# marianaGarcez/SpatialFlink

Measured on AMD Instinct MI355X. Metric: points/sec per window (kNN k=50, range r) at 1/2/4/8 MI355X; % HBM roofline, higher is better.
Workload: dtype f64

## Files before the change

### spatialflink_amd/csrc/gf_internal.hpp

```cpp
#pragma once

#include <hip/hip_runtime.h>

#include <cstdint>
#include <string>
#include <vector>

#include "../../include/geoflink_hip.h"
#include "gf_text.hpp"
#include "gf_numerics.hpp"

struct gf_ctx {
  int device = 0;
  hipStream_t stream = nullptr;
  hipStream_t own_stream = nullptr;
  std::string last_error;
  int timing = 0;
  int timing_period = 1;
  int64_t timing_seq[GF_K_COUNT] = {};
  struct Ev { hipEvent_t a, b; int kid; };
  std::vector<Ev> pending;
  std::vector<hipEvent_t> pool;
  double acc_ms[GF_K_COUNT] = {};
  int64_t acc_n[GF_K_COUNT] = {};
// ... 131 lines not shown
};

struct KnnSampleArgs {
  const double* x;
  const double* y;
  int64_t n;
  double qx, qy;
  QueryRect qr;
  double r, s_r;
  int32_t k;
  int metric;
  int use_hint;
  KnnState* st;
};

struct PolyView {
  const int32_t* ring_off;
  const int32_t* vert_off;
  const double* vx;
  const double* vy;
  const double* ring_env;
  int metric;
  const uint8_t* rect;
};

struct KnnPolyArgs {
  const double* x;
  const double* y;
  const int64_t* objID;
  int64_t begin, end;
  QueryRect qr;
  PolyView poly;
  double bbox[4];
  int approx;
  double r;
  int32_t k;
  int use_state;
  int use_hint;
  KnnState* st;
  double* cand_d;
  uint32_t* cand_i;
  int64_t* cand_o;
  unsigned long long cap;
  uint32_t* maybe_i;
};

struct KnnSelectArgs {
  KnnState* st;
  const double* cand_d;
  const uint32_t* cand_i;
  const int64_t* cand_o;
  unsigned long long cap;
  int use_state;
  double T;
  double r;
  int32_t k;
  int write_hint;
  int64_t idx_base;
  void* result;
};

constexpr int kRangeMaxParts = 4096;
constexpr int kRangeTicketSlot = 2 * kRangeMaxParts;

struct RangeArgs {
  const double* x;
// ... 335 lines not shown
  int64_t* c_maxLen;
  int64_t* c_maxKey;
  int64_t* all_key;
  int64_t* all_len;
};
hipError_t launch_tagg(gf_ctx* ctx, int stage, const TaggArgs& a);

hipError_t launch_knn_sample(gf_ctx* ctx, const KnnSampleArgs& a);
hipError_t launch_knn_scan(gf_ctx* ctx, const KnnScanArgs& a, int blocks, int unroll, int nt);
hipError_t launch_knn_select(gf_ctx* ctx, const KnnSelectArgs& a);
struct KnnLargeArgs {
  const double* cd;
  const int64_t* co;
  const uint32_t* ci;
  uint32_t* perm;
  int64_t m;
  int field;
  uint32_t* keys;
  uint32_t* out;
  uint32_t* cnt;
  int pass;
  unsigned long long* lane_count;
  unsigned long long* lane_maybe;
  int32_t k;
  double T;
  int64_t idx_base;
  void* result;
};
hipError_t launch_knn_large(gf_ctx* ctx, int op, const KnnLargeArgs& a);
constexpr int32_t kMaxKLarge = 1 << 24;
int knn_exact_record(gf_knn_plan* P, const gf_points* pts, void* result);

hipError_t launch_knn_poly_sample(gf_ctx* ctx, const KnnPolyArgs& a);
hipError_t launch_knn_poly_scan(gf_ctx* ctx, const KnnPolyArgs& a, int blocks);
struct KnnSelectArgs;
struct KnnMergeArgs;
hipError_t launch_knn_poly_fused(gf_ctx* ctx, const KnnPolyArgs& a, const KnnSelectArgs& prev, int has_prev,
                                 int blocks, const KnnMergeArgs* merge);
__host__ __device__ inline size_t merge_any_hash(int64_t e) {
  size_t h = 1024;
  while (h < 2 * (size_t)e) h <<= 1;
  return h;
}
__host__ __device__ inline size_t merge_any_bytes(int32_t nrec, int32_t k) {
  const int64_t e = (int64_t)nrec * k;
  return ((size_t)e * 24 + merge_any_hash(e) * 12 + 255) & ~(size_t)255;
}
hipError_t launch_knn_merge(gf_ctx* ctx, int32_t k, const void* records, int32_t nrec, size_t rec_stride,
                            int32_t nwin, size_t win_stride, void* result, size_t res_stride, int foreign,
                            void* scratch);
__host__ __device__ inline size_t str_side_off(int32_t k) { return ((size_t)4 * (k + 1) + 7) & ~(size_t)7; }
__host__ __device__ inline size_t str_record_bytes(int32_t k, int64_t cap) {
  return 32 + (size_t)24 * k + 16 + str_side_off(k) + (((size_t)cap + 7) & ~(size_t)7);
}
__host__ __device__ inline size_t strmerge_pow2(int64_t e) {
  size_t p = 2;
  while (p < (size_t)e) p <<= 1;
  return p;
}
__host__ __device__ inline size_t strmerge_bytes(int32_t nrec, int32_t k) {
  const int64_t e = (int64_t)nrec * k;
  return ((size_t)e * 40 + strmerge_pow2(e) * 4 + strmerge_pow2(2 * e) * 8 + (size_t)k * 16 + 1024) & ~(size_t)255;
}
hipError_t launch_knn_attach_strings(gf_ctx* ctx, int32_t k, const unsigned long long* idmap, const char* arena,
                                     int64_t dict_size, const void* records, int32_t nrec, int64_t cap, void* out);
hipError_t launch_knn_merge_strings(gf_ctx* ctx, int32_t k, int64_t cap, const void* records, int32_t nrec,
                                    size_t rec_stride, int32_t nwin, size_t win_stride, void* results, void* scratch);
constexpr int kMaxMergeRecs = 64;
struct KnnRecList {
  const char* rec[kMaxMergeRecs];
};
// ... 233 lines not shown
  gf_grid grid{};
  double qx = 0, qy = 0, r = 0;
  int32_t k = 0;
  int metric = 0;
  gf::QueryRect qr{};
  struct Lane {
    gf::KnnState* st = nullptr;
    double* cand_d = nullptr;
    uint32_t* cand_i = nullptr;
    int64_t* cand_o = nullptr;
  } lane[6];
  int64_t cap = 0;
  int pipeline = 1;
  uint64_t seq = 0;
  int pend_lane = -1;
  int lane_warm[6] = {0, 0, 0, 0, 0, 0};
  void* pend_result = nullptr;
  int64_t pend_idx_base = 0;
  struct Pend {
    int lane;
    void* result;
    int64_t idx_base;
    uint64_t seq;
  };
  Pend pq[3];
  int npq = 0;
  int use_hint = 1;
  int64_t idx_base = 0;
  void* tmp_result = nullptr;
  void* host_result = nullptr;
  int scan_blocks = 0;
  int scan_unroll = 2;
  int scan_nt = 1;
  int large = 0;
  int poly = 0, approx = 0;
  int32_t* ring_off = nullptr;
  int32_t* vert_off = nullptr;
  double* vx = nullptr;
  double* vy = nullptr;
  double* ring_env = nullptr;
  double bbox[4] = {0, 0, 0, 0};
  uint32_t* maybe_i[3] = {nullptr, nullptr, nullptr};
  int64_t maybe_cap = 0;
};

struct gf_window {
  gf_ctx* ctx = nullptr;
  int64_t capacity = 0, n = 0;
  double* x = nullptr;
  double* y = nullptr;
  int64_t* objID = nullptr;
  int64_t* ts = nullptr;
  bool has_objid = false, has_ts = false;
  const int64_t* objid_mapped = nullptr;
  hipStream_t copy = nullptr;
  hipEvent_t ready = nullptr, fence_main = nullptr, fence_aux = nullptr, fence_aux2 = nullptr;
  bool pending = false;
};
```

### spatialflink_amd/csrc/k_knn.hip

```cpp
#define GF_TU_NAME k_knn_hip
#include "gf_buildtag.hpp"

#include <type_traits>

#include "gf_geom.hpp"
#include "gf_internal.hpp"

namespace gf {

__device__ __forceinline__ bool classify_cg(const QueryRect& q, double px, double py) {
  const double xs = (px == px) ? px : q.minX;
  const double ys = (py == py) ? py : q.minY;
  const bool inG = q.g_any && in_iv(q.gx, xs) && in_iv(q.gy, ys);
  return inG || (in_iv(q.cgx, xs) && in_iv(q.cgy, ys));
}

template <int METRIC>
__device__ __forceinline__ bool knn_pass(double qx, double qy, const QueryRect& qr, double px, double py,
                                         double sp, double T) {
  const double dx = qx - px, dy = qy - py;
  const double s = dx * dx + dy * dy;
  if (!(s <= sp)) return false;
  if (!classify_cg(qr, px, py)) return false;
  return METRIC == 0 ? true : fdlibm_hypot(dx, dy) <= T;
// ... 1126 lines not shown
  for (int j = threadIdx.x; j < kDistBins; j += kBlock) lh[j] = 0u;
  __syncthreads();
  const int64_t n = a.end - a.begin;
  const int64_t stride = n / gridDim.x;
  const int64_t p0 = a.begin + (int64_t)blockIdx.x * stride;
  const int64_t bbase = dist_bin_base(a.r);
  for (int u = threadIdx.x; u < kSamplePerBlock; u += kBlock) {
    const double px = a.x[p0 + u], py = a.y[p0 + u];
    double d;
    if (poly_pass(a, px, py, a.r, d)) atomicAdd(&lh[dist_bin(d, bbase)], 1u);
  }
  sample_finish(a.st, lh, a.k, a.r, a.poly.metric, bbase);
}

__device__ __forceinline__ bool poly_maybe(const KnnPolyArgs& a, double px, double py, double T) {
  if (!classify_cg(a.qr, px, py)) return false;
  return !(px == px && py == py && env_far(a.bbox, px, py, T));
}

__device__ __forceinline__ void maybe_append(const KnnPolyArgs& a, bool c, int64_t i) {
  const uint64_t m = __ballot(c);
  if (m == 0) return;
  const int lane = threadIdx.x & 63;
  const int leader = __ffsll((unsigned long long)m) - 1;
  unsigned long long base = 0;
  if (lane == leader) base = atomicAdd(&a.st->maybe, (unsigned long long)__popcll(m));
  base = __shfl(base, leader, 64);
  if (c) {
    const unsigned long long pos = base + (unsigned long long)__popcll(m & ((1ull << lane) - 1ull));
    if (pos < a.cap) a.maybe_i[pos] = (uint32_t)i;
  }
}

__device__ __forceinline__ void knn_poly_scan_body(const KnnPolyArgs& a, double T, int64_t bid, int64_t nblk) {
  const int lane = threadIdx.x & 63;
  const int64_t stride = nblk * kBlock;
  const int64_t pb = a.begin >> 1, pe = a.end >> 1;
  for (int64_t p = pb + bid * kBlock + threadIdx.x; p - lane < pe; p += stride) {
    const bool in = p < pe;
    dbl2 xv = {0.0, 0.0}, yv = {0.0, 0.0};
    if (in) {
      xv = __builtin_nontemporal_load(reinterpret_cast<const dbl2*>(a.x) + p);
      yv = __builtin_nontemporal_load(reinterpret_cast<const dbl2*>(a.y) + p);
    }
    const bool c0 = in && poly_maybe(a, xv.x, yv.x, T);
    const bool c1 = in && poly_maybe(a, xv.y, yv.y, T);
    if (__ballot(c0 || c1) == 0) continue;
    maybe_append(a, c0, 2 * p);
    maybe_append(a, c1, 2 * p + 1);
  }
  if ((a.end & 1) && bid == 0 && threadIdx.x < 64) {
    const int64_t i = a.end - 1;
    maybe_append(a, lane == 0 && poly_maybe(a, a.x[i], a.y[i], T), i);
  }
}

__global__ __launch_bounds__(kBlock) void knn_poly_scan_kernel(KnnPolyArgs a) {
  knn_poly_scan_body(a, a.use_state ? a.st->T : a.r, blockIdx.x, gridDim.x);
}

__global__ __launch_bounds__(kBlock) void knn_poly_fused_kernel(KnnPolyArgs a, KnnSelectArgs prev, int has_prev,
                                                                KnnMergeArgs m) {
  __shared__ SelLite L;
  if (blockIdx.x == 0) {
    if (has_prev) knn_select_body<SelLite, false>(prev, L);
    if (m.nrec > 0) {
      __threadfence();
      __syncthreads();
      const ListRecs src{&m.list};
      knn_merge_body(prev.k, src, m.nrec, m.result, L);
    }
    return;
  }
  double T;
  if (a.use_state == 2) {
    T = a.st->T;
  } else {
    const double h = a.st->hint_T;
    T = (h > 0.0 && h < a.r) ? h : a.r;
    if (blockIdx.x == 1 && threadIdx.x == 0) a.st->T = T;
  }
  knn_poly_scan_body(a, T, blockIdx.x - 1, gridDim.x - 1);
}

__global__ __launch_bounds__(kBlock) void knn_poly_refine_kernel(KnnPolyArgs a) {
  const double T = a.use_state ? a.st->T : a.r;
  const unsigned long long nm = a.st->maybe;
  if (nm > a.cap) {
    if (blockIdx.x == 0 && threadIdx.x == 0) atomicAdd(&a.st->count, nm);
    return;
  }
  const int lane = threadIdx.x & 63;
  const int64_t stride = (int64_t)gridDim.x * kBlock;
  for (int64_t j = (int64_t)blockIdx.x * kBlock + threadIdx.x; j - lane < (int64_t)nm; j += stride) {
    const bool in = j < (int64_t)nm;
    const int64_t i = in ? (int64_t)a.maybe_i[j] : 0;
    double d = 0.0;
    bool c = false;
    if (in) {
      const double px = a.x[i], py = a.y[i];
      d = a.approx ? point_bbox_distance(px, py, a.bbox) : polygon_distance(px, py, a.poly, 0);
      c = d <= T;
    }
    const uint64_t m = __ballot(c);
    if (m == 0) continue;
    const int leader = __ffsll((unsigned long long)m) - 1;
    unsigned long long base = 0;
    if (lane == leader) base = atomicAdd(&a.st->count, (unsigned long long)__popcll(m));
    base = __shfl(base, leader, 64);
    if (c) {
      const unsigned long long pos = base + (unsigned long long)__popcll(m & ((1ull << lane) - 1ull));
      if (pos < a.cap) {
        a.cand_d[pos] = d;
        a.cand_i[pos] = (uint32_t)i;
        a.cand_o[pos] = a.objID[i];
      }
    }
  }
}

hipError_t launch_knn_poly_sample(gf_ctx* ctx, const KnnPolyArgs& a) {
  KTimer t(ctx, GF_K_KNN_SAMPLE);
  hipLaunchKernelGGL(knn_poly_sample_kernel, dim3(kSampleBlocks), dim3(kBlock), 0, ctx->stream, a);
  return hipGetLastError();
}

hipError_t launch_knn_poly_fused(gf_ctx* ctx, const KnnPolyArgs& a, const KnnSelectArgs& prev, int has_prev,
                                 int blocks, const KnnMergeArgs* merge) {
  KnnMergeArgs m{};
  if (merge && has_prev) m = *merge;
  {
    KTimer t(ctx, GF_K_KNN_SCAN);
    hipLaunchKernelGGL(knn_poly_fused_kernel, dim3(blocks + 1), dim3(kBlock), 0, ctx->stream, a, prev, has_prev, m);
  }
  KnnPolyArgs r = a;
  r.use_state = 1;
  hipLaunchKernelGGL(knn_poly_refine_kernel, dim3(256), dim3(kBlock), 0, ctx->stream, r);
  return hipGetLastError();
}

hipError_t launch_knn_poly_scan(gf_ctx* ctx, const KnnPolyArgs& a, int blocks) {
  {
    KTimer t(ctx, GF_K_KNN_SCAN);
    hipLaunchKernelGGL(knn_poly_scan_kernel, dim3(blocks), dim3(kBlock), 0, ctx->stream, a);
  }
  hipLaunchKernelGGL(knn_poly_refine_kernel, dim3(256), dim3(kBlock), 0, ctx->stream, a);
  return hipGetLastError();
}

struct StrSide {
  int32_t status;
  int32_t n;
  int64_t nbytes;
};
__device__ __forceinline__ StrSide* side_of(void* rec, int32_t k) {
  return reinterpret_cast<StrSide*>((char*)rec + 32 + (size_t)24 * k);
}
__device__ __forceinline__ uint32_t* side_off(void* rec, int32_t k) { return reinterpret_cast<uint32_t*>(side_of(rec, k) + 1); }
__device__ __forceinline__ char* side_bytes(void* rec, int32_t k) { return (char*)side_off(rec, k) + str_side_off(k); }
__device__ __forceinline__ bool dict_key(int64_t o) { return o < GF_OBJID_NUMERIC_MIN; }

template <int NT>
__device__ __forceinline__ uint32_t block_excl(uint32_t v, uint32_t* excl, uint32_t* ws) {
  const int lane = threadIdx.x & 63, w = threadIdx.x >> 6;
  uint32_t inc = v;
#pragma unroll
  for (int o = 1; o < 64; o <<= 1) {
    const uint32_t t = __shfl_up(inc, o, 64);
    if (lane >= o) inc += t;
  }
  if (lane == 63) ws[w] = inc;
  __syncthreads();
  uint32_t before = 0, tot = 0;
#pragma unroll
  for (int i = 0; i < NT / 64; ++i) {
    before += i < w ? ws[i] : 0u;
    tot += ws[i];
  }
  *excl = before + inc - v;
  __syncthreads();
  return tot;
// ... 228 lines not shown
```

### spatialflink_amd/csrc/knn.cpp

```cpp
#define GF_TU_NAME knn_cpp
#include "gf_buildtag.hpp"

#include <hip/hip_runtime.h>

#include <initializer_list>
#include <iterator>
#include <limits>
#include <unordered_set>

#include "gf_host.hpp"

using namespace gf;

extern "C" size_t gf_knn_result_bytes(int32_t k) {
  return sizeof(gf_knn_header) + (size_t)(k > 0 ? k : 0) * (sizeof(double) + 2 * sizeof(int64_t));
}

extern "C" void gf_knn_plan_destroy(gf_knn_plan* P) {
  if (!P) return;
  hipSetDevice(P->ctx->device);
  hipStreamSynchronize(P->ctx->stream);
  for (auto& L : P->lane) {
    if (L.st) hipFree(L.st);
    if (L.cand_d) hipFree(L.cand_d);
// ... 88 lines not shown
    double mnx = poly->vx[v0], mxx = mnx, mny = poly->vy[v0], mxy = mny;
    for (int32_t v = v0 + 1; v < v1; ++v) {
      mnx = std::min(mnx, poly->vx[v]); mxx = std::max(mxx, poly->vx[v]);
      mny = std::min(mny, poly->vy[v]); mxy = std::max(mxy, poly->vy[v]);
    }
    renv[4 * j] = mnx; renv[4 * j + 1] = mxx; renv[4 * j + 2] = mny; renv[4 * j + 3] = mxy;
  }
  P->bbox[0] = renv[0]; P->bbox[1] = renv[2]; P->bbox[2] = renv[1]; P->bbox[3] = renv[3];
  const int32_t gl = guaranteed_layers(g->cellLength, r), cl = candidate_layers(g->cellLength, r);
  const int64_t bx0 = cell_index(P->bbox[0], g->minX, g->cellLength), bx1 = cell_index(P->bbox[2], g->minX, g->cellLength);
  const int64_t by0 = cell_index(P->bbox[1], g->minY, g->cellLength), by1 = cell_index(P->bbox[3], g->minY, g->cellLength);
  const double nan = std::numeric_limits<double>::quiet_NaN();
  const int64_t n1 = g->n - 1;
  QueryRect q;
  q.minX = g->minX;
  q.minY = g->minY;
  if (cl > 0) {
    q.cgx = axis_iv(std::max<int64_t>(bx0 - cl, 0), std::min<int64_t>(bx1 + cl, n1), g->minX, g->cellLength);
    q.cgy = axis_iv(std::max<int64_t>(by0 - cl, 0), std::min<int64_t>(by1 + cl, n1), g->minY, g->cellLength);
  } else {
    q.cgx = q.cgy = {nan, nan};
  }
  if (gl > 0) {
    q.gx = axis_iv(std::max<int64_t>(bx0 - gl, 0), std::min<int64_t>(bx1 + gl, n1), g->minX, g->cellLength);
    q.gy = axis_iv(std::max<int64_t>(by0 - gl, 0), std::min<int64_t>(by1 + gl, n1), g->minY, g->cellLength);
  } else if (gl == 0) {
    q.gx = axis_iv(bx0, bx1, g->minX, g->cellLength);
    q.gy = axis_iv(by0, by1, g->minY, g->cellLength);
  } else {
    q.gx = q.gy = {nan, nan};
  }
  q.g_any = (gl >= 0) && !std::isnan(q.gx.lo) && !std::isnan(q.gy.lo);
  P->qr = q;
  const int32_t nverts = poly->vert_off[nrings];
  std::vector<int32_t> ro = {0, nrings}, vo(poly->vert_off, poly->vert_off + nrings + 1);
  std::vector<double> vx(poly->vx, poly->vx + nverts), vy(poly->vy, poly->vy + nverts);
  if ((st = upload(ctx, &P->ring_off, ro)) || (st = upload(ctx, &P->vert_off, vo)) || (st = upload(ctx, &P->vx, vx)) ||
      (st = upload(ctx, &P->vy, vy)) || (st = upload(ctx, &P->ring_env, renv))) {
    gf_knn_plan_destroy(P);
    return st;
  }
  *out = P;
  return GF_OK;
}

extern "C" int gf_knn_plan_set_capacity(gf_knn_plan* P, int64_t cap) {
  if (!P || cap < 2 || cap > (int64_t)1 << 31) return GF_ERR_ARG;
  int st = bind(P->ctx);
  if (st) return st;
  int fs = gf_knn_plan_flush(P);
  if (fs) return fs;
  hipStreamSynchronize(P->ctx->stream);
  return knn_alloc_candidates(P, cap & ~(int64_t)1);
}

extern "C" int gf_knn_plan_set_tuning(gf_knn_plan* P, int32_t scan_blocks, int32_t unroll, int32_t nontemporal) {
  if (!P || scan_blocks < 0 || unroll < 1 || unroll > 8) return GF_ERR_ARG;
  P->scan_blocks = scan_blocks;
  P->scan_unroll = unroll;
  P->scan_nt = nontemporal != 0;
  return GF_OK;
}

extern "C" int gf_knn_plan_set_index_base(gf_knn_plan* P, int64_t base) {
  if (!P || base < 0) return GF_ERR_ARG;
  P->idx_base = base;
  return GF_OK;
}

static int scan_blocks_for(gf_knn_plan* P, int64_t n) {
  int blocks = P->scan_blocks;
  if (blocks <= 0) {
    blocks = stream_blocks(P->ctx, (n + 1) / 2);
    blocks = std::min(blocks, P->ctx->num_cus * 4);
  }
  return blocks;
}

static KnnScanArgs scan_args(gf_knn_plan* P, int j, const gf_points* pts, int64_t begin, int64_t end, int use_state) {
  const gf_knn_plan::Lane& L = P->lane[j];
  KnnScanArgs s{};
  s.x = pts->x; s.y = pts->y; s.objID = pts->objID; s.begin = begin; s.end = end;
  s.qx = P->qx; s.qy = P->qy; s.qr = P->qr;
  s.T = P->r; s.s_pre = s_prefilter(P->r, P->metric);
  s.use_state = use_state; s.metric = P->metric; s.st = L.st;
  s.cand_d = L.cand_d; s.cand_i = L.cand_i; s.cand_o = L.cand_o; s.cap = (unsigned long long)P->cap;
  return s;
}

static KnnSelectArgs select_args(gf_knn_plan* P, int j, int use_state, int write_hint, void* result,
                                 int64_t idx_base) {
  const gf_knn_plan::Lane& L = P->lane[j];
  KnnSelectArgs q{};
  q.st = L.st; q.cand_d = L.cand_d; q.cand_i = L.cand_i; q.cand_o = L.cand_o;
  q.cap = (unsigned long long)P->cap;
  q.use_state = use_state; q.T = P->r; q.r = P->r; q.k = P->k; q.result = result;
  q.write_hint = write_hint; q.idx_base = idx_base;
  return q;
}

static KnnPolyArgs poly_args(gf_knn_plan* P, int j, const gf_points* pts, int64_t begin, int64_t end, int use_state,
                             int use_hint) {
  const gf_knn_plan::Lane& L = P->lane[j];
  KnnPolyArgs a{};
  a.x = pts->x; a.y = pts->y; a.objID = pts->objID; a.begin = begin; a.end = end;
  a.qr = P->qr;
  a.poly = PolyView{P->ring_off, P->vert_off, P->vx, P->vy, P->ring_env, P->metric};
  for (int i = 0; i < 4; ++i) a.bbox[i] = P->bbox[i];
  a.approx = P->approx; a.r = P->r; a.k = P->k; a.use_state = use_state; a.use_hint = use_hint;
  a.st = L.st; a.cand_d = L.cand_d; a.cand_i = L.cand_i; a.cand_o = L.cand_o; a.cap = (unsigned long long)P->cap;
  a.maybe_i = P->maybe_i[P->pipeline >= 3 ? j % (P->pipeline - 1) : j];
  return a;
}

static int poly_buffers(gf_knn_plan* P) {
  if (P->maybe_cap >= P->cap) return GF_OK;
  GF_HIP_CHECK(P->ctx, hipStreamSynchronize(P->ctx->stream));
  if (int e = sync_aux(P->ctx)) return e;
  for (auto& m : P->maybe_i) {
    if (m) hipFree(m);
    m = nullptr;
    GF_HIP_CHECK(P->ctx, hipMalloc(&m, sizeof(uint32_t) * (size_t)P->cap));
  }
  P->maybe_cap = P->cap;
  return GF_OK;
}

static int knn_scan_select(gf_knn_plan* P, int j, const gf_points* pts, int64_t begin, int64_t end, int use_state,
                           int write_hint, void* result) {
  gf_ctx* ctx = P->ctx;
  if (P->poly) {
    int st = poly_buffers(P);
    if (st) return st;
    const KnnPolyArgs a = poly_args(P, j, pts, begin, end, use_state, 0);
    GF_HIP_CHECK(ctx, launch_knn_poly_scan(ctx, a, scan_blocks_for(P, (end - begin + 1) / 2)));
    GF_HIP_CHECK(ctx, launch_knn_select(ctx, select_args(P, j, use_state, write_hint, result, P->idx_base)));
    return GF_OK;
  }
  const KnnScanArgs s = scan_args(P, j, pts, begin, end, use_state);
  GF_HIP_CHECK(ctx, launch_knn_scan(ctx, s, scan_blocks_for(P, end - begin), P->scan_unroll, P->scan_nt));
  GF_HIP_CHECK(ctx, launch_knn_select(ctx, select_args(P, j, use_state, write_hint, result, P->idx_base)));
  return GF_OK;
}

static int knn_large(gf_knn_plan* P, const gf_points* pts, void* result) {
  gf_ctx* ctx = P->ctx;
  int st;
  const int64_t n = pts->n;
  if (P->cap < n && (st = knn_alloc_candidates(P, n))) return st;
  if (P->poly) {
    if ((st = poly_buffers(P))) return st;
    GF_HIP_CHECK(ctx, launch_knn_poly_scan(ctx, poly_args(P, 0, pts, 0, n, 0, 0), scan_blocks_for(P, (n + 1) / 2)));
  } else {
    const KnnScanArgs s = scan_args(P, 0, pts, 0, n, 0);
    GF_HIP_CHECK(ctx, launch_knn_scan(ctx, s, scan_blocks_for(P, n), P->scan_unroll, P->scan_nt));
  }
  const gf_knn_plan::Lane& L = P->lane[0];
  const int64_t mm = std::max<int64_t>(n, 1);
  const int nb = radix_blocks(ctx, mm);
  const int64_t mat = (int64_t)256 * nb;
  Arena ar;
  uint32_t *keys[2], *perm[2], *cnt, *m, *ms;
  ar.take(keys[0], mm); ar.take(keys[1], mm);
  ar.take(perm[0], mm); ar.take(perm[1], mm);
  ar.take(cnt, 2); ar.take(m, mat); ar.take(ms, mat + 1);
  if ((st = ar.alloc(ctx))) return st;
  KnnLargeArgs a{};
  a.cd = L.cand_d; a.co = L.cand_o; a.ci = L.cand_i; a.k = P->k; a.T = P->r; a.idx_base = P->idx_base;
  a.result = result; a.m = mm; a.cnt = cnt;
  a.lane_count = &L.st->count; a.lane_maybe = &L.st->maybe;
  GF_HIP_CHECK(ctx, launch_knn_large(ctx, 5, a));
  int cur = 0;
  auto sort_by = [&](int pass, std::initializer_list<int> fields) -> int {
    for (int f : fields) {
      a.perm = perm[cur]; a.field = f; a.keys = keys[0]; a.pass = pass;
      GF_HIP_CHECK(ctx, launch_knn_large(ctx, 1, a));
      for (int p = 0; p < 4; ++p) {
        RadixArgs r{};
        r.tile = radix_tile();
        r.n = mm; r.n_dev = a.cnt + pass;
        r.kin = keys[p & 1]; r.vin = perm[cur];
        r.kout = keys[(p + 1) & 1]; r.vout = perm[cur ^ 1];
        r.shift = p * 8; r.bits = 8; r.nblk = nb; r.M = m; r.Ms = ms;
        GF_HIP_CHECK(ctx, launch_radix(ctx, 0, r, nb));
        if (int e = scan1(ctx, m, mat, ms)) return e;
// ... 51 lines not shown
    const uint64_t kseq = P->seq++;
    const int S = P->pipeline >= 3 ? P->pipeline - 1 : 1, j = (int)(kseq % (uint64_t)S);
    hipStream_t main = ctx->stream;
    ctx->stream = knn_stream(ctx, main, j);
    const bool staged = pts->n >= kSampleMinN;
    int rc = staged ? knn_launch_sample(P, j, pts, P->use_hint) : GF_OK;
    if (rc == GF_OK) rc = knn_scan_select(P, j, pts, 0, pts->n, staged ? 1 : 0, staged && P->use_hint, result);
    ctx->stream = main;
    return rc;
  }
  if (P->pipeline >= 3) {
    if (P->poly && (st = poly_buffers(P))) return st;
    const uint64_t S = (uint64_t)(P->pipeline - 1), kseq = P->seq++;
    const int j = (int)(kseq % (2 * S));
    hipStream_t main = ctx->stream;
    ctx->stream = knn_stream(ctx, main, (int)(kseq % S));
    int rc = GF_OK;
    do {
      const bool sample = pts->n >= kSampleMinN && (!P->use_hint || !P->lane_warm[j]);
      if (sample && (rc = knn_launch_sample(P, j, pts, 0))) break;
      P->lane_warm[j] = 1;
      KnnSelectArgs q{};
      int has_prev = 0;
      if (P->npq > 0 && P->pq[0].seq + S == kseq) {
        const gf_knn_plan::Pend e = P->pq[0];
        q = select_args(P, e.lane, 1, P->use_hint, e.result, e.idx_base);
        has_prev = 1;
        for (int t = 1; t < P->npq; ++t) P->pq[t - 1] = P->pq[t];
        --P->npq;
      }
      hipError_t he;
      if (P->poly)
        he = launch_knn_poly_fused(ctx, poly_args(P, j, pts, 0, pts->n, sample ? 2 : 1, 0), q, has_prev,
                                   scan_blocks_for(P, (pts->n + 1) / 2), nullptr);
      else
        he = launch_knn_fused(ctx, scan_args(P, j, pts, 0, pts->n, sample ? 2 : 1), q, has_prev,
                              scan_blocks_for(P, pts->n), P->scan_unroll, P->scan_nt, merge);
      if (he != hipSuccess) { rc = hip_err(ctx, he, "launch_knn_fused"); break; }
      P->pq[P->npq++] = gf_knn_plan::Pend{j, result, P->idx_base, kseq};
    } while (0);
    ctx->stream = main;
    return rc;
  }
  if (P->pipeline == 2) {
    const int j = (int)(P->seq++ & 1);
    if (P->poly && (st = poly_buffers(P))) return st;
    const bool sample = pts->n >= kSampleMinN && (!P->use_hint || !P->lane_warm[j]);
    if (sample && (st = knn_launch_sample(P, j, pts, 0))) return st;
    P->lane_warm[j] = 1;
    const int use_state = sample ? 2 : 1;
    KnnSelectArgs q{};
    const int has_prev = P->pend_lane >= 0;
    if (has_prev) q = select_args(P, P->pend_lane, 1, P->use_hint, P->pend_result, P->pend_idx_base);
    const bool fold = merge && merge->nrec > 0 && has_prev && P->k <= kFusedMergeMaxK;
    if (P->poly)
      GF_HIP_CHECK(ctx, launch_knn_poly_fused(ctx, poly_args(P, j, pts, 0, pts->n, use_state, 0), q, has_prev,
                                             scan_blocks_for(P, (pts->n + 1) / 2), fold ? merge : nullptr));
    else
      GF_HIP_CHECK(ctx, launch_knn_fused(ctx, scan_args(P, j, pts, 0, pts->n, use_state), q, has_prev,
                                         scan_blocks_for(P, pts->n), P->scan_unroll, P->scan_nt,
                                         fold ? merge : nullptr));
    *merged = fold ? 1 : 0;
    P->pend_lane = j;
    P->pend_result = result;
    P->pend_idx_base = P->idx_base;
    return GF_OK;
  }
  const bool staged = pts->n >= kSampleMinN;
  if (staged && (st = knn_launch_sample(P, 0, pts, P->use_hint))) return st;
  return knn_scan_select(P, 0, pts, 0, pts->n, staged ? 1 : 0, staged && P->use_hint, result);
}

extern "C" int gf_knn_plan_flush(gf_knn_plan* P) {
  if (!P) return GF_ERR_ARG;
  if (P->pipeline >= 3) {
    if (P->npq == 0) return P->k > kFusedSelectMaxK ? gf_ctx_join(P->ctx) : GF_OK;
    gf_ctx* ctx = P->ctx;
    int st = bind(ctx);
    if (st) return st;
    hipStream_t main = ctx->stream;
    for (int e = 0; e < P->npq; ++e) {
      const gf_knn_plan::Pend& w = P->pq[e];
      ctx->stream = knn_stream(ctx, main, (int)(w.seq % (uint64_t)(P->pipeline - 1)));
      hipError_t he = launch_knn_select(ctx, select_args(P, w.lane, 1, P->use_hint, w.result, w.idx_base));
      ctx->stream = main;
      if (he != hipSuccess) return hip_err(ctx, he, "launch_knn_select");
    }
    P->npq = 0;
    return gf_ctx_join(ctx);
  }
// ... 182 lines not shown
```

Before: 768.7 billion.

## Filter polygon kNN scan on x first, loading y only for surviving lanes

The polygon kNN scan now checks each point's x coordinate against the query grid intervals and the polygon bbox band before loading y. It only issues y loads for tiles where some lane survives, which cuts HBM reads when x alone rejects most points. The scan body is also templated on an unroll factor and a nontemporal flag, with software prefetch of the next x tile. When T equals the full radius r, it falls back to the old path that loads both coordinates. The x-band test uses a small relative slack, so correctness depends on that tolerance staying conservative.

```diff
diff --git a/spatialflink_amd/csrc/gf_internal.hpp b/spatialflink_amd/csrc/gf_internal.hpp
--- a/spatialflink_amd/csrc/gf_internal.hpp
+++ b/spatialflink_amd/csrc/gf_internal.hpp
@@ -588,11 +588,11 @@
 int knn_exact_record(gf_knn_plan* P, const gf_points* pts, void* result);
 
 hipError_t launch_knn_poly_sample(gf_ctx* ctx, const KnnPolyArgs& a);
-hipError_t launch_knn_poly_scan(gf_ctx* ctx, const KnnPolyArgs& a, int blocks);
+hipError_t launch_knn_poly_scan(gf_ctx* ctx, const KnnPolyArgs& a, int blocks, int unroll, int nt);
 struct KnnSelectArgs;
 struct KnnMergeArgs;
 hipError_t launch_knn_poly_fused(gf_ctx* ctx, const KnnPolyArgs& a, const KnnSelectArgs& prev, int has_prev,
-                                 int blocks, const KnnMergeArgs* merge);
+                                 int blocks, int unroll, int nt, const KnnMergeArgs* merge);
 __host__ __device__ inline size_t merge_any_hash(int64_t e) {
   size_t h = 1024;
   while (h < 2 * (size_t)e) h <<= 1;
@@ -892,6 +892,8 @@
   int scan_blocks = 0;
   int scan_unroll = 2;
   int scan_nt = 1;
+  int poly_unroll = 1;
+  int poly_nt = 0;
   int large = 0;
   int poly = 0, approx = 0;
   int32_t* ring_off = nullptr;
diff --git a/spatialflink_amd/csrc/k_knn.hip b/spatialflink_amd/csrc/k_knn.hip
--- a/spatialflink_amd/csrc/k_knn.hip
+++ b/spatialflink_amd/csrc/k_knn.hip
@@ -1182,7 +1182,56 @@
   }
 }
 
-__device__ __forceinline__ void knn_poly_scan_body(const KnnPolyArgs& a, double T, int64_t bid, int64_t nblk) {
+struct PolyBand {
+  double T1;
+  double S;
+};
+__device__ __forceinline__ PolyBand poly_band(const KnnPolyArgs& a, double T) {
+  PolyBand b;
+  b.T1 = T * (1.0 + 1e-8);
+  b.S = fabs(a.bbox[0]) + fabs(a.bbox[1]) + fabs(a.bbox[2]) + fabs(a.bbox[3]);
+  return b;
+}
+__device__ __forceinline__ bool poly_x_maybe(const KnnPolyArgs& a, const PolyBand& b, double px) {
+  const bool num = px == px;
+  const double xs = num ? px : a.qr.minX;
+  if (!in_iv(a.qr.cgx, xs) && !(a.qr.g_any && in_iv(a.qr.gx, xs))) return false;
+  const double dx = px < a.bbox[0] ? a.bbox[0] - px : (px > a.bbox[2] ? px - a.bbox[2] : 0.0);
+  return !(num && dx > b.T1 + (fabs(px) + b.S) * 1e-11);
+}
+__device__ __forceinline__ uint32_t poly_x_mask(const KnnPolyArgs& a, const PolyBand& b, const dbl2& xv) {
+  return (uint32_t)poly_x_maybe(a, b, xv.x) | ((uint32_t)poly_x_maybe(a, b, xv.y) << 1);
+}
+
+template <int U, int NT>
+__device__ __forceinline__ void knn_poly_tile_x(const KnnPolyArgs& a, const PolyBand& b, const dbl2 (&xv)[U],
+                                                const dbl2* py, int64_t p0, int64_t wstride, double T) {
+  uint32_t xm = 0;
+#pragma unroll
+  for (int u = 0; u < U; ++u) xm |= poly_x_mask(a, b, xv[u]) << (2 * u);
+  if (__ballot(xm != 0) == 0) return;
+  dbl2 yv[U];
+#pragma unroll
+  for (int u = 0; u < U; ++u) {
+    yv[u].x = 0.0; yv[u].y = 0.0;
+    if ((xm >> (2 * u)) & 3u) yv[u] = ld2<NT>(py + u * wstride);
+  }
+  uint32_t cm = 0;
+#pragma unroll
+  for (int u = 0; u < U; ++u) {
+    if ((xm >> (2 * u)) & 1u) cm |= (uint32_t)poly_maybe(a, xv[u].x, yv[u].x, T) << (2 * u);
+    if ((xm >> (2 * u)) & 2u) cm |= (uint32_t)poly_maybe(a, xv[u].y, yv[u].y, T) << (2 * u + 1);
+  }
+  if (__ballot(cm != 0) == 0) return;
+#pragma unroll
+  for (int u = 0; u < U; ++u) {
+    const int64_t i0 = 2 * (p0 + u * wstride);
+    maybe_append(a, (cm >> (2 * u)) & 1u, i0);
+    maybe_append(a, (cm >> (2 * u + 1)) & 1u, i0 + 1);
+  }
+}
+
+__device__ __forceinline__ void knn_poly_scan_both(const KnnPolyArgs& a, double T, int64_t bid, int64_t nblk) {
   const int lane = threadIdx.x & 63;
   const int64_t stride = nblk * kBlock;
   const int64_t pb = a.begin >> 1, pe = a.end >> 1;
@@ -1199,16 +1248,67 @@
     maybe_append(a, c0, 2 * p);
     maybe_append(a, c1, 2 * p + 1);
   }
+}
+
+template <int U, int NT>
+__device__ __forceinline__ void knn_poly_scan_body(const KnnPolyArgs& a, double T, int64_t bid, int64_t nblk) {
+  const int lane = threadIdx.x & 63;
+  const int64_t wstride = nblk * kBlock;
+  const int64_t pbeg = a.begin >> 1, pe = a.end >> 1;
+  const int64_t iters = (pe - pbeg) / (U * wstride);
+  const int64_t off = bid * kBlock + threadIdx.x;
+  const dbl2* px = reinterpret_cast<const dbl2*>(a.x) + pbeg + off;
+  const dbl2* py = reinterpret_cast<const dbl2*>(a.y) + pbeg + off;
+  const PolyBand b = poly_band(a, T);
+  const bool wide = T == a.r;
+  if (wide) knn_poly_scan_both(a, T, bid, nblk);
+  dbl2 xv[U];
+  if (!wide && iters > 0) {
+#pragma unroll
+    for (int u = 0; u < U; ++u) xv[u] = ld2<NT>(px + u * wstride);
+  }
+  for (int64_t it = 0; !wide && it < iters; ++it) {
+    dbl2 xn[U];
+    px += U * wstride;
+    if (it + 1 < iters) {
+#pragma unroll
+      for (int u = 0; u < U; ++u) xn[u] = ld2<NT>(px + u * wstride);
+    } else {
+#pragma unroll
+      for (int u = 0; u < U; ++u) { xn[u].x = 0.0; xn[u].y = 0.0; }
+    }
+    knn_poly_tile_x<U, NT>(a, b, xv, py, pbeg + off + it * U * wstride, wstride, T);
+    py += U * wstride;
+#pragma unroll
+    for (int u = 0; u < U; ++u) xv[u] = xn[u];
+  }
+  for (int64_t p = pbeg + iters * U * wstride + off; !wide && p - lane < pe; p += wstride) {
+    dbl2 xt = {0.0, 0.0}, yt = {0.0, 0.0};
+    uint32_t xm = 0;
+    if (p < pe) {
+      xt = *(reinterpret_cast<const dbl2*>(a.x) + p);
+      xm = poly_x_mask(a, b, xt);
+    }
+    if (__ballot(xm != 0) == 0) continue;
+    if (xm) yt = *(reinterpret_cast<const dbl2*>(a.y) + p);
+    const bool c0 = (xm & 1u) && poly_maybe(a, xt.x, yt.x, T);
+    const bool c1 = (xm & 2u) && poly_maybe(a, xt.y, yt.y, T);
+    if (__ballot(c0 || c1) == 0) continue;
+    maybe_append(a, c0, 2 * p);
+    maybe_append(a, c1, 2 * p + 1);
+  }
   if ((a.end & 1) && bid == 0 && threadIdx.x < 64) {
     const int64_t i = a.end - 1;
     maybe_append(a, lane == 0 && poly_maybe(a, a.x[i], a.y[i], T), i);
   }
 }
 
+template <int U, int NT>
 __global__ __launch_bounds__(kBlock) void knn_poly_scan_kernel(KnnPolyArgs a) {
-  knn_poly_scan_body(a, a.use_state ? a.st->T : a.r, blockIdx.x, gridDim.x);
-}
-
+  knn_poly_scan_body<U, NT>(a, a.use_state ? a.st->T : a.r, blockIdx.x, gridDim.x);
+}
+
+template <int U, int NT>
 __global__ __launch_bounds__(kBlock) void knn_poly_fused_kernel(KnnPolyArgs a, KnnSelectArgs prev, int has_prev,
                                                                 KnnMergeArgs m) {
   __shared__ SelLite L;
@@ -1230,7 +1330,7 @@
     T = (h > 0.0 && h < a.r) ? h : a.r;
     if (blockIdx.x == 1 && threadIdx.x == 0) a.st->T = T;
   }
-  knn_poly_scan_body(a, T, blockIdx.x - 1, gridDim.x - 1);
+  knn_poly_scan_body<U, NT>(a, T, blockIdx.x - 1, gridDim.x - 1);
 }
 
 __global__ __launch_bounds__(kBlock) void knn_poly_refine_kernel(KnnPolyArgs a) {
@@ -1276,12 +1376,19 @@
 }
 
 hipError_t launch_knn_poly_fused(gf_ctx* ctx, const KnnPolyArgs& a, const KnnSelectArgs& prev, int has_prev,
-                                 int blocks, const KnnMergeArgs* merge) {
+                                 int blocks, int unroll, int nt, const KnnMergeArgs* merge) {
   KnnMergeArgs m{};
   if (merge && has_prev) m = *merge;
   {
     KTimer t(ctx, GF_K_KNN_SCAN);
-    hipLaunchKernelGGL(knn_poly_fused_kernel, dim3(blocks + 1), dim3(kBlock), 0, ctx->stream, a, prev, has_prev, m);
+    const dim3 g(blocks + 1), b(kBlock);
+#define GF_PFUSED(U, N) hipLaunchKernelGGL((knn_poly_fused_kernel<U, N>), g, b, 0, ctx->stream, a, prev, has_prev, m)
+    if (nt) {
+      if (unroll <= 1) GF_PFUSED(1, 1); else if (unroll == 2) GF_PFUSED(2, 1); else GF_PFUSED(4, 1);
+    } else {
+      if (unroll <= 1) GF_PFUSED(1, 0); else if (unroll == 2) GF_PFUSED(2, 0); else GF_PFUSED(4, 0);
+    }
+#undef GF_PFUSED
   }
   KnnPolyArgs r = a;
   r.use_state = 1;
@@ -1289,10 +1396,17 @@
   return hipGetLastError();
 }
 
-hipError_t launch_knn_poly_scan(gf_ctx* ctx, const KnnPolyArgs& a, int blocks) {
+hipError_t launch_knn_poly_scan(gf_ctx* ctx, const KnnPolyArgs& a, int blocks, int unroll, int nt) {
   {
     KTimer t(ctx, GF_K_KNN_SCAN);
-    hipLaunchKernelGGL(knn_poly_scan_kernel, dim3(blocks), dim3(kBlock), 0, ctx->stream, a);
+    const dim3 g(blocks), b(kBlock);
+#define GF_PSCAN(U, N) hipLaunchKernelGGL((knn_poly_scan_kernel<U, N>), g, b, 0, ctx->stream, a)
+    if (nt) {
+      if (unroll <= 1) GF_PSCAN(1, 1); else if (unroll == 2) GF_PSCAN(2, 1); else GF_PSCAN(4, 1);
+    } else {
+      if (unroll <= 1) GF_PSCAN(1, 0); else if (unroll == 2) GF_PSCAN(2, 0); else GF_PSCAN(4, 0);
+    }
+#undef GF_PSCAN
   }
   hipLaunchKernelGGL(knn_poly_refine_kernel, dim3(256), dim3(kBlock), 0, ctx->stream, a);
   return hipGetLastError();
diff --git a/spatialflink_amd/csrc/knn.cpp b/spatialflink_amd/csrc/knn.cpp
--- a/spatialflink_amd/csrc/knn.cpp
+++ b/spatialflink_amd/csrc/knn.cpp
@@ -170,7 +170,9 @@
   if (!P || scan_blocks < 0 || unroll < 1 || unroll > 8) return GF_ERR_ARG;
   P->scan_blocks = scan_blocks;
   P->scan_unroll = unroll;
+  P->poly_unroll = unroll;
   P->scan_nt = nontemporal != 0;
+  P->poly_nt = P->scan_nt;
   return GF_OK;
 }
 
@@ -245,7 +247,8 @@
     int st = poly_buffers(P);
     if (st) return st;
     const KnnPolyArgs a = poly_args(P, j, pts, begin, end, use_state, 0);
-    GF_HIP_CHECK(ctx, launch_knn_poly_scan(ctx, a, scan_blocks_for(P, (end - begin + 1) / 2)));
+    GF_HIP_CHECK(ctx, launch_knn_poly_scan(ctx, a, scan_blocks_for(P, (end - begin + 1) / 2), P->poly_unroll,
+                                           P->poly_nt));
     GF_HIP_CHECK(ctx, launch_knn_select(ctx, select_args(P, j, use_state, write_hint, result, P->idx_base)));
     return GF_OK;
   }
@@ -262,7 +265,8 @@
   if (P->cap < n && (st = knn_alloc_candidates(P, n))) return st;
   if (P->poly) {
     if ((st = poly_buffers(P))) return st;
-    GF_HIP_CHECK(ctx, launch_knn_poly_scan(ctx, poly_args(P, 0, pts, 0, n, 0, 0), scan_blocks_for(P, (n + 1) / 2)));
+    GF_HIP_CHECK(ctx, launch_knn_poly_scan(ctx, poly_args(P, 0, pts, 0, n, 0, 0), scan_blocks_for(P, (n + 1) / 2),
+                                           P->poly_unroll, P->poly_nt));
   } else {
     const KnnScanArgs s = scan_args(P, 0, pts, 0, n, 0);
     GF_HIP_CHECK(ctx, launch_knn_scan(ctx, s, scan_blocks_for(P, n), P->scan_unroll, P->scan_nt));
@@ -380,7 +384,7 @@
       hipError_t he;
       if (P->poly)
         he = launch_knn_poly_fused(ctx, poly_args(P, j, pts, 0, pts->n, sample ? 2 : 1, 0), q, has_prev,
-                                   scan_blocks_for(P, (pts->n + 1) / 2), nullptr);
+                                   scan_blocks_for(P, (pts->n + 1) / 2), P->poly_unroll, P->poly_nt, nullptr);
       else
         he = launch_knn_fused(ctx, scan_args(P, j, pts, 0, pts->n, sample ? 2 : 1), q, has_prev,
                               scan_blocks_for(P, pts->n), P->scan_unroll, P->scan_nt, merge);
@@ -403,7 +407,8 @@
     const bool fold = merge && merge->nrec > 0 && has_prev && P->k <= kFusedMergeMaxK;
     if (P->poly)
       GF_HIP_CHECK(ctx, launch_knn_poly_fused(ctx, poly_args(P, j, pts, 0, pts->n, use_state, 0), q, has_prev,
-                                             scan_blocks_for(P, (pts->n + 1) / 2), fold ? merge : nullptr));
+                                             scan_blocks_for(P, (pts->n + 1) / 2), P->poly_unroll, P->poly_nt,
+                                             fold ? merge : nullptr));
     else
       GF_HIP_CHECK(ctx, launch_knn_fused(ctx, scan_args(P, j, pts, 0, pts->n, use_state), q, has_prev,
                                          scan_blocks_for(P, pts->n), P->scan_unroll, P->scan_nt,
```

After: 769.2 billion (median of 6 runs). About the same (+0.1%).

## Prefilter polygon kNN scan on x before loading y, add unroll/NT variants

Applied to the files above, without the earlier changes.

The polygon kNN scan now loads only the x coordinates first and rejects points whose x-distance to the polygon bbox exceeds the threshold (with a conservative error margin using a y-magnitude cap computed on the host). The y coordinates are loaded only for lanes that survive, which cuts HBM traffic when most points are far away. The scan is also templated on unroll and nontemporal-load choice with software prefetch of the next x tile; the plan sets unroll 1 and nontemporal loads by default. This adds complexity and relies on the conservative margin to keep results exact.

```diff
diff --git a/spatialflink_amd/csrc/gf_internal.hpp b/spatialflink_amd/csrc/gf_internal.hpp
--- a/spatialflink_amd/csrc/gf_internal.hpp
+++ b/spatialflink_amd/csrc/gf_internal.hpp
@@ -187,6 +187,7 @@
   QueryRect qr;
   PolyView poly;
   double bbox[4];
+  double ycap;
   int approx;
   double r;
   int32_t k;
@@ -588,11 +589,11 @@
 int knn_exact_record(gf_knn_plan* P, const gf_points* pts, void* result);
 
 hipError_t launch_knn_poly_sample(gf_ctx* ctx, const KnnPolyArgs& a);
-hipError_t launch_knn_poly_scan(gf_ctx* ctx, const KnnPolyArgs& a, int blocks);
+hipError_t launch_knn_poly_scan(gf_ctx* ctx, const KnnPolyArgs& a, int blocks, int unroll, int nt);
 struct KnnSelectArgs;
 struct KnnMergeArgs;
 hipError_t launch_knn_poly_fused(gf_ctx* ctx, const KnnPolyArgs& a, const KnnSelectArgs& prev, int has_prev,
-                                 int blocks, const KnnMergeArgs* merge);
+                                 int blocks, int unroll, int nt, const KnnMergeArgs* merge);
 __host__ __device__ inline size_t merge_any_hash(int64_t e) {
   size_t h = 1024;
   while (h < 2 * (size_t)e) h <<= 1;
@@ -900,6 +901,7 @@
   double* vy = nullptr;
   double* ring_env = nullptr;
   double bbox[4] = {0, 0, 0, 0};
+  double ycap = 0;
   uint32_t* maybe_i[3] = {nullptr, nullptr, nullptr};
   int64_t maybe_cap = 0;
 };
diff --git a/spatialflink_amd/csrc/k_knn.hip b/spatialflink_amd/csrc/k_knn.hip
--- a/spatialflink_amd/csrc/k_knn.hip
+++ b/spatialflink_amd/csrc/k_knn.hip
@@ -1182,33 +1182,96 @@
   }
 }
 
+__device__ __forceinline__ bool poly_x_reject(const KnnPolyArgs& a, double px, double T) {
+  const double* bb = a.bbox;
+  const double dx = px < bb[0] ? bb[0] - px : (px > bb[2] ? px - bb[2] : 0.0);
+  const double scaleY = fabs(px) + a.ycap + fabs(bb[0]) + fabs(bb[1]) + fabs(bb[2]) + fabs(bb[3]);
+  const double rmY = T + T * 1e-9 + scaleY * 1e-12;
+  return px == px && dx > rmY;
+}
+
+__device__ __forceinline__ uint32_t poly_keep(const KnnPolyArgs& a, const dbl2& xv, double T) {
+  return (uint32_t)!poly_x_reject(a, xv.x, T) | ((uint32_t)!poly_x_reject(a, xv.y, T) << 1);
+}
+
+template <int U, int NT>
+__device__ __forceinline__ void knn_poly_tile_x(const KnnPolyArgs& a, const dbl2 (&xv)[U], const uint32_t (&keep)[U],
+                                                const dbl2* py, int64_t p0, int64_t wstride, double T) {
+  uint32_t any = 0;
+#pragma unroll
+  for (int u = 0; u < U; ++u) any |= keep[u];
+  if (__ballot(any != 0) == 0) return;
+  uint32_t cm = 0;
+#pragma unroll
+  for (int u = 0; u < U; ++u) {
+    if (keep[u]) {
+      const dbl2 yv = ld2<NT>(py + u * wstride);
+      if ((keep[u] & 1u) && poly_maybe(a, xv[u].x, yv.x, T)) cm |= 1u << (2 * u);
+      if ((keep[u] & 2u) && poly_maybe(a, xv[u].y, yv.y, T)) cm |= 2u << (2 * u);
+    }
+  }
+  if (__ballot(cm != 0) == 0) return;
+#pragma unroll
+  for (int u = 0; u < U; ++u) {
+    const int64_t i0 = 2 * (p0 + u * wstride);
+    maybe_append(a, (cm >> (2 * u)) & 1u, i0);
+    maybe_append(a, (cm >> (2 * u + 1)) & 1u, i0 + 1);
+  }
+}
+
+template <int U, int NT>
 __device__ __forceinline__ void knn_poly_scan_body(const KnnPolyArgs& a, double T, int64_t bid, int64_t nblk) {
   const int lane = threadIdx.x & 63;
-  const int64_t stride = nblk * kBlock;
+  const int64_t wstride = nblk * kBlock;
   const int64_t pb = a.begin >> 1, pe = a.end >> 1;
-  for (int64_t p = pb + bid * kBlock + threadIdx.x; p - lane < pe; p += stride) {
-    const bool in = p < pe;
-    dbl2 xv = {0.0, 0.0}, yv = {0.0, 0.0};
-    if (in) {
-      xv = __builtin_nontemporal_load(reinterpret_cast<const dbl2*>(a.x) + p);
-      yv = __builtin_nontemporal_load(reinterpret_cast<const dbl2*>(a.y) + p);
-    }
-    const bool c0 = in && poly_maybe(a, xv.x, yv.x, T);
-    const bool c1 = in && poly_maybe(a, xv.y, yv.y, T);
-    if (__ballot(c0 || c1) == 0) continue;
-    maybe_append(a, c0, 2 * p);
-    maybe_append(a, c1, 2 * p + 1);
+  const int64_t iters = (pe - pb) / (U * wstride);
+  const int64_t off = bid * kBlock + threadIdx.x;
+  const dbl2* px = reinterpret_cast<const dbl2*>(a.x) + pb + off;
+  const dbl2* py = reinterpret_cast<const dbl2*>(a.y) + pb + off;
+  dbl2 xv[U];
+  if (iters > 0) {
+#pragma unroll
+    for (int u = 0; u < U; ++u) xv[u] = ld2<NT>(px + u * wstride);
+  }
+  for (int64_t it = 0; it < iters; ++it) {
+    dbl2 xn[U];
+    px += U * wstride;
+    if (it + 1 < iters) {
+#pragma unroll
+      for (int u = 0; u < U; ++u) xn[u] = ld2<NT>(px + u * wstride);
+    } else {
+#pragma unroll
+      for (int u = 0; u < U; ++u) { xn[u].x = 0.0; xn[u].y = 0.0; }
+    }
+    uint32_t keep[U];
+#pragma unroll
+    for (int u = 0; u < U; ++u) keep[u] = poly_keep(a, xv[u], T);
+    knn_poly_tile_x<U, NT>(a, xv, keep, py, pb + off + it * U * wstride, wstride, T);
+    py += U * wstride;
+#pragma unroll
+    for (int u = 0; u < U; ++u) xv[u] = xn[u];
+  }
+  for (int64_t p = pb + iters * U * wstride + off; p - lane < pe; p += wstride) {
+    dbl2 xt[1] = {{0.0, 0.0}};
+    uint32_t kt[1] = {0u};
+    if (p < pe) {
+      xt[0] = *(reinterpret_cast<const dbl2*>(a.x) + p);
+      kt[0] = poly_keep(a, xt[0], T);
+    }
+    knn_poly_tile_x<1, 0>(a, xt, kt, reinterpret_cast<const dbl2*>(a.y) + p, p, wstride, T);
   }
   if ((a.end & 1) && bid == 0 && threadIdx.x < 64) {
     const int64_t i = a.end - 1;
-    maybe_append(a, lane == 0 && poly_maybe(a, a.x[i], a.y[i], T), i);
-  }
-}
-
+    maybe_append(a, lane == 0 && !poly_x_reject(a, a.x[i], T) && poly_maybe(a, a.x[i], a.y[i], T), i);
+  }
+}
+
+template <int U, int NT>
 __global__ __launch_bounds__(kBlock) void knn_poly_scan_kernel(KnnPolyArgs a) {
-  knn_poly_scan_body(a, a.use_state ? a.st->T : a.r, blockIdx.x, gridDim.x);
-}
-
+  knn_poly_scan_body<U, NT>(a, a.use_state ? a.st->T : a.r, blockIdx.x, gridDim.x);
+}
+
+template <int U, int NT>
 __global__ __launch_bounds__(kBlock) void knn_poly_fused_kernel(KnnPolyArgs a, KnnSelectArgs prev, int has_prev,
                                                                 KnnMergeArgs m) {
   __shared__ SelLite L;
@@ -1230,7 +1293,7 @@
     T = (h > 0.0 && h < a.r) ? h : a.r;
     if (blockIdx.x == 1 && threadIdx.x == 0) a.st->T = T;
   }
-  knn_poly_scan_body(a, T, blockIdx.x - 1, gridDim.x - 1);
+  knn_poly_scan_body<U, NT>(a, T, blockIdx.x - 1, gridDim.x - 1);
 }
 
 __global__ __launch_bounds__(kBlock) void knn_poly_refine_kernel(KnnPolyArgs a) {
@@ -1275,13 +1338,28 @@
   return hipGetLastError();
 }
 
+#define GF_POLY_VARIANTS(KERNEL, ...)                                                   \
+  do {                                                                                  \
+    if (nt) {                                                                           \
+      if (unroll <= 1) GF_POLY_LAUNCH(KERNEL, 1, 1, __VA_ARGS__);                       \
+      else if (unroll == 2) GF_POLY_LAUNCH(KERNEL, 2, 1, __VA_ARGS__);                  \
+      else GF_POLY_LAUNCH(KERNEL, 4, 1, __VA_ARGS__);                                   \
+    } else {                                                                            \
+      if (unroll <= 1) GF_POLY_LAUNCH(KERNEL, 1, 0, __VA_ARGS__);                       \
+      else if (unroll == 2) GF_POLY_LAUNCH(KERNEL, 2, 0, __VA_ARGS__);                  \
+      else GF_POLY_LAUNCH(KERNEL, 4, 0, __VA_ARGS__);                                   \
+    }                                                                                   \
+  } while (0)
+#define GF_POLY_LAUNCH(KERNEL, U, N, ...) hipLaunchKernelGGL((KERNEL<U, N>), g, dim3(kBlock), 0, ctx->stream, __VA_ARGS__)
+
 hipError_t launch_knn_poly_fused(gf_ctx* ctx, const KnnPolyArgs& a, const KnnSelectArgs& prev, int has_prev,
-                                 int blocks, const KnnMergeArgs* merge) {
+                                 int blocks, int unroll, int nt, const KnnMergeArgs* merge) {
   KnnMergeArgs m{};
   if (merge && has_prev) m = *merge;
   {
     KTimer t(ctx, GF_K_KNN_SCAN);
-    hipLaunchKernelGGL(knn_poly_fused_kernel, dim3(blocks + 1), dim3(kBlock), 0, ctx->stream, a, prev, has_prev, m);
+    const dim3 g(blocks + 1);
+    GF_POLY_VARIANTS(knn_poly_fused_kernel, a, prev, has_prev, m);
   }
   KnnPolyArgs r = a;
   r.use_state = 1;
@@ -1289,14 +1367,17 @@
   return hipGetLastError();
 }
 
-hipError_t launch_knn_poly_scan(gf_ctx* ctx, const KnnPolyArgs& a, int blocks) {
+hipError_t launch_knn_poly_scan(gf_ctx* ctx, const KnnPolyArgs& a, int blocks, int unroll, int nt) {
   {
     KTimer t(ctx, GF_K_KNN_SCAN);
-    hipLaunchKernelGGL(knn_poly_scan_kernel, dim3(blocks), dim3(kBlock), 0, ctx->stream, a);
+    const dim3 g(blocks);
+    GF_POLY_VARIANTS(knn_poly_scan_kernel, a);
   }
   hipLaunchKernelGGL(knn_poly_refine_kernel, dim3(256), dim3(kBlock), 0, ctx->stream, a);
   return hipGetLastError();
 }
+#undef GF_POLY_LAUNCH
+#undef GF_POLY_VARIANTS
 
 struct StrSide {
   int32_t status;
diff --git a/spatialflink_amd/csrc/knn.cpp b/spatialflink_amd/csrc/knn.cpp
--- a/spatialflink_amd/csrc/knn.cpp
+++ b/spatialflink_amd/csrc/knn.cpp
@@ -144,6 +144,17 @@
   }
   q.g_any = (gl >= 0) && !std::isnan(q.gx.lo) && !std::isnan(q.gy.lo);
   P->qr = q;
+  double ycap = 0.0;
+  auto widen = [&](const AxisIv& iv) {
+    if (std::isnan(iv.lo)) return;
+    if (std::isnan(iv.hi_excl) || std::isinf(iv.lo) || std::isinf(iv.hi_excl)) { ycap = INFINITY; return; }
+    ycap = std::max(ycap, std::max(std::fabs(iv.lo), std::fabs(iv.hi_excl)));
+  };
+  widen(q.cgy);
+  if (q.g_any) widen(q.gy);
+  P->ycap = ycap;
+  P->scan_unroll = 1;
+  P->scan_nt = 1;
   const int32_t nverts = poly->vert_off[nrings];
   std::vector<int32_t> ro = {0, nrings}, vo(poly->vert_off, poly->vert_off + nrings + 1);
   std::vector<double> vx(poly->vx, poly->vx + nverts), vy(poly->vy, poly->vy + nverts);
@@ -219,6 +230,7 @@
   a.qr = P->qr;
   a.poly = PolyView{P->ring_off, P->vert_off, P->vx, P->vy, P->ring_env, P->metric};
   for (int i = 0; i < 4; ++i) a.bbox[i] = P->bbox[i];
+  a.ycap = P->ycap;
   a.approx = P->approx; a.r = P->r; a.k = P->k; a.use_state = use_state; a.use_hint = use_hint;
   a.st = L.st; a.cand_d = L.cand_d; a.cand_i = L.cand_i; a.cand_o = L.cand_o; a.cap = (unsigned long long)P->cap;
   a.maybe_i = P->maybe_i[P->pipeline >= 3 ? j % (P->pipeline - 1) : j];
@@ -245,7 +257,7 @@
     int st = poly_buffers(P);
     if (st) return st;
     const KnnPolyArgs a = poly_args(P, j, pts, begin, end, use_state, 0);
-    GF_HIP_CHECK(ctx, launch_knn_poly_scan(ctx, a, scan_blocks_for(P, (end - begin + 1) / 2)));
+    GF_HIP_CHECK(ctx, launch_knn_poly_scan(ctx, a, scan_blocks_for(P, (end - begin + 1) / 2), P->scan_unroll, P->scan_nt));
     GF_HIP_CHECK(ctx, launch_knn_select(ctx, select_args(P, j, use_state, write_hint, result, P->idx_base)));
     return GF_OK;
   }
@@ -262,7 +274,8 @@
   if (P->cap < n && (st = knn_alloc_candidates(P, n))) return st;
   if (P->poly) {
     if ((st = poly_buffers(P))) return st;
-    GF_HIP_CHECK(ctx, launch_knn_poly_scan(ctx, poly_args(P, 0, pts, 0, n, 0, 0), scan_blocks_for(P, (n + 1) / 2)));
+    GF_HIP_CHECK(ctx, launch_knn_poly_scan(ctx, poly_args(P, 0, pts, 0, n, 0, 0), scan_blocks_for(P, (n + 1) / 2),
+                                           P->scan_unroll, P->scan_nt));
   } else {
     const KnnScanArgs s = scan_args(P, 0, pts, 0, n, 0);
     GF_HIP_CHECK(ctx, launch_knn_scan(ctx, s, scan_blocks_for(P, n), P->scan_unroll, P->scan_nt));
@@ -380,7 +393,7 @@
       hipError_t he;
       if (P->poly)
         he = launch_knn_poly_fused(ctx, poly_args(P, j, pts, 0, pts->n, sample ? 2 : 1, 0), q, has_prev,
-                                   scan_blocks_for(P, (pts->n + 1) / 2), nullptr);
+                                   scan_blocks_for(P, (pts->n + 1) / 2), P->scan_unroll, P->scan_nt, nullptr);
       else
         he = launch_knn_fused(ctx, scan_args(P, j, pts, 0, pts->n, sample ? 2 : 1), q, has_prev,
                               scan_blocks_for(P, pts->n), P->scan_unroll, P->scan_nt, merge);
@@ -403,7 +416,8 @@
     const bool fold = merge && merge->nrec > 0 && has_prev && P->k <= kFusedMergeMaxK;
     if (P->poly)
       GF_HIP_CHECK(ctx, launch_knn_poly_fused(ctx, poly_args(P, j, pts, 0, pts->n, use_state, 0), q, has_prev,
-                                             scan_blocks_for(P, (pts->n + 1) / 2), fold ? merge : nullptr));
+                                             scan_blocks_for(P, (pts->n + 1) / 2), P->scan_unroll, P->scan_nt,
+                                             fold ? merge : nullptr));
     else
       GF_HIP_CHECK(ctx, launch_knn_fused(ctx, scan_args(P, j, pts, 0, pts->n, use_state), q, has_prev,
                                          scan_blocks_for(P, pts->n), P->scan_unroll, P->scan_nt,
```

After: 753.7 billion before, 756.4 billion after, median of 4. Within noise of the previous version (+0.4%).
